# tho-kn/EgoTAP

Measured on AMD Instinct MI355X. Metric: stereo frames/sec (2D->3D lift, B=256, 256x256), higher is better.
Workload: dtype f32; 1 GPU; UnrealEgo 16-joint lifting head (heatmaps [B,90,64,64] -> joints [B,16,3]), forward only, fp32, batch 256 per GPU, inputs resident in HBM; batch_per_gpu=256, global_batch=256, heatmap=64, parallelism=dp1 (batch shards, no collective)

## Files before the change

### egotap_amd/csrc/egotap_abi.hip

```cpp
#include <stdarg.h>
#include <stdio.h>
#include <string.h>

#include <string>
#include <unordered_map>
#include <vector>

#include "attention_f32.h"
#include "common.h"
#include "conv_f32.h"
#include "conv_bf16.h"
#include "gemm_f32.h"
#include "gemm_bf16.h"
#include "gemm_bf16_dma.h"
#include "gemm_f32_dma.h"
#include "attention_bf16.h"
#include "layernorm.h"
#include "metrics.h"
#include "heatmap_synth.h"
#include "pu_chain.h"
#include "gemm_tn_bf16.h"
#include "train_ops.h"
#include "gemm_bf16s.h"
#include "gemm_bf16s64.h"
// ... 82 lines not shown
    const float *x2f0_w, *x2f0_b, *x2h0_w, *x2h0_b, *b2h0_w, *b2h0_b, *h2h0_w, *h2h0_b;
    const float *x2f1_w, *x2f1_b, *x2h1_w, *x2h1_b, *h2h1_w, *h2h1_b;
    const float *pose_w, *pose_b, *glob_w, *glob_b;
};

struct HmParams {
    struct Bn { const float *g, *b, *m, *v; long long* nbt; };
    const float* stem_w; Bn stem_bn;
    struct Block { const float *w1, *w2, *wd; Bn bn1, bn2, bnd; } blk[4][6];
    int nblk[4];
    struct Cv { const float *w, *b; } l1x1[4], up[3], head;
    int n_out;
};

struct egotap_handle_s {
    egotap_config cfg;
    int J, T, grid, ppd, side, seq, C, D, H, hid, out_joints;
    std::unordered_map<std::string, int64_t> expect[EGOTAP_NET_COUNT];
    std::unordered_map<std::string, Param> bound[EGOTAP_NET_COUNT];
    bool lift_resolved = false;
    LiftParams lp;
    std::unordered_map<std::string, Param> bound_grad;
    bool grad_resolved = false;
    LiftParams lg;
    bool hm_resolved[EGOTAP_NET_COUNT] = {false, false, false};
    HmParams hp[EGOTAP_NET_COUNT];
    int debug_stop = 0;
    int pu_resident[2] = {-1, -1};
    bool pu_chain = true;
    unsigned* pu_fault_host = nullptr;
    unsigned* pu_fault_dev = nullptr;
    int pu_faults = 0;
    int pu_debug_drop = 0;
    int precision = EGOTAP_PREC_F32;
    __bf16* wscratch = nullptr;
    size_t wscratch_bytes = 0;
    __bf16* ascratch = nullptr;
    size_t ascratch_bytes = 0;
    __bf16* conv_pack = nullptr;
    float* conv_part = nullptr;
    size_t conv_part_floats = 0;
    char* lift_arena = nullptr;
    char* hm_arena[EGOTAP_NET_COUNT] = {nullptr, nullptr, nullptr};
    short hm_arena_slab[EGOTAP_NET_COUNT][PackTable::MAXW] = {};
    int hm_arena_nw[EGOTAP_NET_COUNT] = {0, 0, 0};
    bool timing = false;
    std::vector<hipEvent_t> ev;
    struct Rec { const char* role; const char* kernel; double flops; };
    std::vector<Rec> rec;
    size_t ev_used = 0;
    std::string detail;
};
typedef egotap_handle_s Handle;

static int isqrt_floor(int v) {
    int r = 0;
    while ((r + 1) * (r + 1) <= v) ++r;
    return r;
}

static void lift_expect(Handle* h) {
    auto& e = h->expect[EGOTAP_NET_LIFT];
    const int64_t D = h->D, H = h->H, hid = h->hid, x = 2 * hid;
    const std::string v = "pos_heatmap_encoder.vit.";
    e[v + "embeddings.mask_token"] = D;
    e[v + "embeddings.position_embeddings"] = (int64_t)h->seq * D;
// ... 273 lines not shown
#endif
#if EGOTAP_IN(0)
extern "C" const char* egotap_timing_detail(egotap_handle h) { return h ? h->detail.c_str() : ""; }
#endif

struct GemmTimer {
    Handle* h;
    hipStream_t s;
    bool on;
    GemmTimer(Handle* h_, hipStream_t s_, const char* role, const char* kernel, double flops)
        : h(h_), s(s_), on(h_ && h_->timing) {
        if (!on) return;
        if (h->ev_used + 2 > h->ev.size()) {
            hipEvent_t a, b;
            if (hipEventCreate(&a) != hipSuccess || hipEventCreate(&b) != hipSuccess) { on = false; return; }
            h->ev.push_back(a);
            h->ev.push_back(b);
        }
        (void)hipEventRecord(h->ev[h->ev_used], s);
        h->rec.push_back({role, kernel, flops});
    }
    ~GemmTimer() {
        if (!on) return;
        (void)hipEventRecord(h->ev[h->ev_used + 1], s);
        h->ev_used += 2;
    }
};

template <class AL> struct AlName;
template <> struct AlName<ALoadPlain> { static constexpr const char* v = "ALoadPlain"; };
template <> struct AlName<ALoadPatch> { static constexpr const char* v = "ALoadPatch"; };
template <> struct AlName<ALoadTokens> { static constexpr const char* v = "ALoadTokens"; };
template <> struct AlName<ALoadLive> { static constexpr const char* v = "ALoadLive"; };
template <> struct AlName<ALoadRot> { static constexpr const char* v = "ALoadRot"; };
template <> struct AlName<ALoadStereo> { static constexpr const char* v = "ALoadStereo"; };
template <> struct AlName<ALoadStereoGated> { static constexpr const char* v = "ALoadStereoGated"; };
template <class E> struct EpiName;
template <> struct EpiName<EpiBias> { static constexpr const char* v = "EpiBias"; };
template <> struct EpiName<EpiBiasRes> { static constexpr const char* v = "EpiBiasRes"; };
template <> struct EpiName<EpiBiasResLive> { static constexpr const char* v = "EpiBiasResLive"; };
template <> struct EpiName<EpiBiasGelu> { static constexpr const char* v = "EpiBiasGelu"; };
template <> struct EpiName<EpiBnLrelu> { static constexpr const char* v = "EpiBnLrelu"; };
template <> struct EpiName<EpiPatch> { static constexpr const char* v = "EpiPatch"; };

template <class Cfg, class AL, class Epi>
static hipError_t gemm(Handle* h, const char* role, const AL& al, const SegMat& W, const Epi& epi, float* C, long ldc,
                       int M, int N, int K, hipStream_t s) {
    static const std::string kname = std::string("gemm_f32_kernel<") + std::to_string(Cfg::BM) + "x" +
                                     std::to_string(Cfg::BN) + "x" + std::to_string(Cfg::BK) + "," + AlName<AL>::v + "," +
                                     EpiName<Epi>::v + ">";
    GemmTimer t(h, s, role, kname.c_str(), 2.0 * M * N * K);
    return gemm_f32_launch<Cfg, AL, Epi>(al, W, epi, C, ldc, M, N, K, s);
}

static int device_cu_count() {
    static int n = 0;
    if (n == 0) {
        int dev = 0, v = 0;
        if (hipGetDevice(&dev) == hipSuccess && hipDeviceGetAttribute(&v, hipDeviceAttributeMultiprocessorCount, dev) == hipSuccess && v > 0) n = v;
        else n = 256;
    }
    return n;
}

static __global__ __launch_bounds__(256) void zero_fill_kernel(f32x4* __restrict__ p, long n16) {
    const long i = (long)blockIdx.x * blockDim.x + threadIdx.x;
    if (i < n16) p[i] = f32x4{0.f, 0.f, 0.f, 0.f};
}
static hipError_t zero_fill(void* p, size_t bytes, hipStream_t s) {
    if (bytes == 0) return hipSuccess;
    if ((((uintptr_t)p) | bytes) & 15) return hipErrorInvalidValue;
    const long n16 = (long)(bytes / 16);
    hipLaunchKernelGGL(zero_fill_kernel, dim3((unsigned)((n16 + 255) / 256)), dim3(256), 0, s, (f32x4*)p, n16);
    return hipGetLastError();
}

static __global__ __launch_bounds__(256) void concat3_kernel(const float* __restrict__ a, const float* __restrict__ b, const float* __restrict__ c,
                                                             float* __restrict__ out, int n) {
    const int i = blockIdx.x * blockDim.x + threadIdx.x;
    if (i < n) { out[i] = a[i]; out[n + i] = b[i]; out[2 * n + i] = c[i]; }
}

static __global__ __launch_bounds__(256) void f32_to_bf16_rows_kernel(const float* __restrict__ src, long lda, __bf16* __restrict__ dst, int k8, long n8) {
    const long i = (long)blockIdx.x * blockDim.x + threadIdx.x;
    if (i >= n8) return;
    const long row = i / k8;
    const float* p = src + row * lda + (i - row * k8) * 8;
    *(bf16x8*)(dst + i * 8) = bf16_round8(*(const f32x4*)p, *(const f32x4*)(p + 4));
}
template <class AL, class Epi>
static hipError_t gemm_bf16_plain(Handle* h, const AL& al, const SegMat& W, const Epi& epi, float* C, long ldc, int M, int N, int K, hipStream_t s) {
    const int nseg = N / W.seg;
    if (h && h->wscratch && (size_t)N * K * 2 <= h->wscratch_bytes && K % 8 == 0 && W.ld == K && nseg >= 1 && nseg <= 3 && nseg * W.seg == N) {
        SegMatB B;
        for (int i = 0; i < 3; ++i) B.p[i] = h->wscratch + (size_t)(i < nseg ? i : 0) * W.seg * K;
        B.seg = W.seg; B.ld = K;
        const long n8 = (long)W.seg * K / 8;
        for (int i = 0; i < nseg; ++i)
            hipLaunchKernelGGL(f32_to_bf16_kernel, dim3((unsigned)((n8 + 255) / 256)), dim3(256), 0, s, W.p[i], h->wscratch + (size_t)i * W.seg * K, n8);
        hipError_t e = hipGetLastError();
        if (e != hipSuccess) return e;
        if constexpr (std::is_same<AL, ALoadPlain>::value) {
            if (K % DmaCfg::BK == 0 && N % DmaCfg::BN == 0 && W.seg % DmaCfg::BN == 0 && al.lda % 4 == 0 && M >= 1024) {
                __bf16* a = (size_t)M * K * 2 <= h->ascratch_bytes ? h->ascratch : nullptr;
                if (a) {
                    const long a8 = (long)M * K / 8;
// ... 171 lines not shown
    EGO_CHECK(B >= 0, "negative batch");
    *bytes = lift_ws(h, B > 0 ? B : 1).total;
    return EGOTAP_OK;
}
#endif

#if EGOTAP_IN(0)
extern "C" int egotap_lift_intermediate(egotap_handle h, int B, const char* name, size_t* offset, int64_t* numel) {
    EGO_CHECK(h && name && offset && numel, "null argument");
    const LiftWs w = lift_ws(h, B > 0 ? B : 1);
    const int64_t M = (int64_t)B * h->seq;
    if (!strcmp(name, "tokens")) { *offset = w.Y; *numel = M * h->D; }
    else if (!strcmp(name, "x")) { *offset = w.X; *numel = M * h->D; }
    else if (!strcmp(name, "pos_embed")) { *offset = w.POSZ; *numel = (int64_t)B * h->T * h->hid; }
    else if (!strcmp(name, "rot_embed")) { *offset = w.ROTZ; *numel = (int64_t)B * h->T * h->hid; }
    else if (!strcmp(name, "skel_embed")) { *offset = w.HS1; *numel = (int64_t)h->J * B * h->H; }
    else { egotap_set_error("unknown intermediate '%s'", name); return EGOTAP_ERR_INVALID; }
    return EGOTAP_OK;
}
#endif

#if EGOTAP_IN(0)
extern "C" int egotap_set_pu_chain(egotap_handle h, int enable) {
    EGO_CHECK(h, "null handle");
    h->pu_chain = enable != 0;
    h->pu_resident[0] = h->pu_resident[1] = -1;
    return EGOTAP_OK;
}
extern "C" int egotap_debug_pu_drop_workgroups(egotap_handle h, int n) {
    EGO_CHECK(h && n >= 0 && n < 16, "egotap_debug_pu_drop_workgroups: n in [0, 16)");
    h->pu_debug_drop = n;
    return EGOTAP_OK;
}
extern "C" int egotap_pu_chain_status(egotap_handle h, int* enabled, int* faults) {
    EGO_CHECK(h, "null handle");
    if (h->pu_fault_host && __atomic_load_n(h->pu_fault_host, __ATOMIC_RELAXED) != 0u) {
        __atomic_store_n(h->pu_fault_host, 0u, __ATOMIC_RELAXED);
        h->pu_faults++;
        h->pu_chain = false;
        h->pu_resident[0] = h->pu_resident[1] = -1;
    }
    if (enabled) *enabled = h->pu_chain ? 1 : 0;
    if (faults) *faults = h->pu_faults;
    return EGOTAP_OK;
}
extern "C" int egotap_set_precision(egotap_handle h, int mode) {
    EGO_CHECK(h, "null handle");
    EGO_CHECK(mode == EGOTAP_PREC_F32 || mode == EGOTAP_PREC_BF16X3 || mode == EGOTAP_PREC_BF16, "egotap_set_precision: unknown mode %d", mode);
    h->precision = mode;
    h->lift_arena = nullptr;
    for (int n = 0; n < EGOTAP_NET_COUNT; ++n) h->hm_arena[n] = nullptr;
    return EGOTAP_OK;
}
#endif

#if EGOTAP_IN(0)
extern "C" int egotap_set_weight_scratch(egotap_handle h, void* buf, size_t bytes) {
    EGO_CHECK(h, "null handle");
    EGO_CHECK(((uintptr_t)buf & 15) == 0, "egotap_set_weight_scratch: 16-byte alignment");
    h->wscratch = (__bf16*)buf;
    h->wscratch_bytes = buf ? bytes : 0;
    return EGOTAP_OK;
}
#endif

#if EGOTAP_IN(0)
// ... 67 lines not shown
static EpiBiasResLive rebase(EpiBiasResLive e, int m0) { e.lr.m0 += m0; return e; }
template <class AL, class Epi>
static hipError_t gemm_rounds(Handle* h, const char* role, const AL& al, const SegMat& W, const Epi& epi, float* C, long ldc, int M, int N, int K,
                              hipStream_t s) {
    const int cus = device_cu_count(), tn = N / 256;
    const long tiles = (long)((M + 255) / 256) * tn;
    const int mh = (int)((tiles / cus) * cus / tn) * 256;
    if (N % 256 == 0 && K % 32 == 0 && mh > 0 && mh < M) {
        const double t_round = K * 0.2319 + 5.0;
        const double t_big = (double)((tiles + cus - 1) / cus) * t_round;
        const double t_split = (double)(((long)(mh / 256) * tn + cus - 1) / cus) * t_round + 4.0 + gemm_f32_direct_estimate_us<TileA>(M - mh, N, K, cus);
        if (t_split < t_big) {
            hipError_t e = gemm_big(h, role, al, W, epi, C, ldc, mh, N, K, s);
            if (e != hipSuccess) return e;
            return gemm<TileA>(h, role, rebase(al, mh), W, rebase(epi, mh), C + (long)mh * ldc, ldc, M - mh, N, K, s);
        }
    }
    return gemm_big(h, role, al, W, epi, C, ldc, M, N, K, s);
}

static bool lift_prune_last(Handle* h, int B) {
#ifdef EGOTAP_ATTN_F32_LIVE
    const int D = h->D, M = B * h->seq, Nq = h->T * h->ppd * h->ppd;
    if (h->precision != EGOTAP_PREC_F32 || h->debug_stop != 0 || h->cfg.vit_layers < 1 || Nq < 32 || Nq >= h->seq || D % 256 != 0) return false;
    const int cus = device_cu_count();
    if (gemm_small_route(h, true, M, 3 * D, D, D, cus, true).kind != GS_BIG || gemm_small_route(h, true, M, D, D, D, cus).kind != GS_BIG ||
        gemm_small_route(h, true, M, 4 * D, D, 4 * D, cus, true).kind != GS_BIG || gemm_small_route(h, true, M, D, 4 * D, D, cus).kind != GS_BIG)
        return false;
    return attention_f32_ksplit(B, h->seq, h->cfg.vit_heads, SPLITK_FLOATS, cus) == 1;
#else
    (void)h; (void)B;
    return false;
#endif
}

struct LiftFrozen {
    size_t patch, qkv[8], o[8], up[8], dn[8], bias3[8], fc1p, fc1r, total;
};
static bool lift_frozen_route(const Handle* h) { return h->precision == EGOTAP_PREC_BF16 && h->D == 1024 && h->seq % 32 == 0; }
static LiftFrozen lift_frozen_plan(const Handle* h, const LiftParams* p, PrepTable* T) {
    LiftFrozen f{};
    const size_t D = h->D, K1 = (size_t)h->ppd * h->ppd * D, K1r = 2 * (size_t)h->cfg.hm_size * h->cfg.hm_size;
    const int NL = h->cfg.vit_layers;
    size_t o = 0;
    int ns = 0;
    unsigned chunk = 0;
    auto seg = [&](const float* src, size_t elems, size_t elem_bytes, size_t at) {
        const size_t dst = at == (size_t)-1 ? o : at;
        if (at == (size_t)-1) o = al256(o + elems * elem_bytes);
        if (T && ns < PrepTable::MAXS) {
            T->s[ns] = PrepSeg{src, (unsigned long long)dst, (unsigned)(elems / 8), chunk};
            chunk += (unsigned)((elems / 8 + PrepTable::CHUNK8 - 1) / PrepTable::CHUNK8);
        }
        ++ns;
        return dst;
    };
    const size_t own = (size_t)-1;
    f.patch = seg(p ? p->patch_w : nullptr, D * 256, 2, own);
    for (int i = 0; i < NL; ++i) {
        const LiftParams::Layer* L = p ? &p->layer[i] : nullptr;
        f.qkv[i] = o;
        o = al256(o + 3 * D * D * 2);
        seg(L ? L->q_w : nullptr, D * D, 2, f.qkv[i]);
        seg(L ? L->k_w : nullptr, D * D, 2, f.qkv[i] + D * D * 2);
        seg(L ? L->v_w : nullptr, D * D, 2, f.qkv[i] + 2 * D * D * 2);
        f.o[i] = seg(L ? L->o_w : nullptr, D * D, 2, own);
// ... 101 lines not shown
            if (h->debug_stop == 2 + i) return EGOTAP_OK;
        }
        ln(p.lnf_g, p.lnf_b);
        auto bnf = [](const LiftParams::Fc& f, float* out) { return SEpiBnLreluF32{f.b, f.g, f.beta, f.mean, f.var, 1e-5f, 0.2f, out, 2048L}; };
        auto bn = [](const LiftParams::Fc& f) { return EpiBnLrelu{f.b, f.g, f.beta, f.mean, f.var, 1e-5f, 0.2f}; };
        {
            const int K1 = h->ppd * h->ppd * D;
            if (!frozen) prep(p.pos_fc[0].w, Wb, 2048, K1);
            const __bf16* W1 = frozen ? FW(fz.fc1p) : Wb;
            const XTokens xt{Yb, h->T, D, h->seq, h->side, h->ppd, h->grid};
            const int sp = gemm_bf16s_ksplit(BT, 2048, K1, cu, SPLITK_FLOATS);
            if (sp > 1) EGO_HIP(gemm_bf16s_splitk_launch(xt, W1, (long)K1, bnf(p.pos_fc[0], Z1), SPK, sp, BT, 2048, K1, cu, s));
            else EGO_HIP(fc1_nt(h, 0, Yb, W1, (long)K1, bnf(p.pos_fc[0], Z1), BT, cu, s));
            EGO_HIP((fc_gemm(h, "pos_fc2", ALoadPlain{Z1, 2048}, segmat1(p.pos_fc[1].w, 512, 2048), bn(p.pos_fc[1]), Z2, 512, BT, 512, 2048, SPK, s)));
            EGO_HIP((fc_gemm(h, "pos_fc3", ALoadPlain{Z2, 512}, segmat1(p.pos_fc[2].w, hid, 512), bn(p.pos_fc[2]), POSZ, hid, BT, hid, 512, SPK, s)));
        }
        {
            __bf16* hmb = HIDb;
            const long n8 = (long)B * h->C * HW / 8;
            hipLaunchKernelGGL(f32_to_bf16_kernel, dim3((unsigned)((n8 + 255) / 256)), dim3(256), 0, s, hm, hmb, n8);
            if (!frozen) prep(p.rot_fc[0].w, Wb, 2048, 2 * HW);
            const __bf16* W1 = frozen ? FW(fz.fc1r) : Wb;
            EGO_HIP(hipGetLastError());
            const XRot xr{hmb, h->C, J, HW};
            const int sp = gemm_bf16s_ksplit(BT, 2048, 2 * HW, cu, SPLITK_FLOATS);
            if (sp > 1) EGO_HIP(gemm_bf16s_splitk_launch(xr, W1, 2L * HW, bnf(p.rot_fc[0], Z1), SPK, sp, BT, 2048, 2 * HW, cu, s));
            else EGO_HIP(fc1_nt(h, 1, hmb, W1, 2L * HW, bnf(p.rot_fc[0], Z1), BT, cu, s));
            EGO_HIP((fc_gemm(h, "rot_fc2", ALoadPlain{Z1, 2048}, segmat1(p.rot_fc[1].w, 512, 2048), bn(p.rot_fc[1]), Z2, 512, BT, 512, 2048, SPK, s)));
            EGO_HIP((fc_gemm(h, "rot_fc3", ALoadPlain{Z2, 512}, segmat1(p.rot_fc[2].w, hid, 512), bn(p.rot_fc[2]), ROTZ, hid, BT, hid, 512, SPK, s)));
        }
    } else {
    const int NL = h->cfg.vit_layers;
    const bool prune = pose_only && lift_prune_last(h, B);
    EGO_HIP(launch_ln(X, Y, NL > 0 ? p.layer[0].ln1_g : p.lnf_g, NL > 0 ? p.layer[0].ln1_b : p.lnf_b, M, 1e-12f, s));
    for (int i = 0; i < NL; ++i) {
        const auto& L = p.layer[i];
#ifdef EGOTAP_ATTN_F32_LIVE
        if (prune && i + 1 == NL) {
            const LiveRows lr{h->seq, h->side, h->ppd, h->grid, h->T};
            const int Nq = h->T * h->ppd * h->ppd, Mc = B * Nq;
            float* Xc = QKV;
            SegMat Wkv; Wkv.p[0] = L.k_w; Wkv.p[1] = L.v_w; Wkv.p[2] = L.v_w; Wkv.seg = D; Wkv.ld = D;
            SegVec bkv; bkv.p[0] = L.k_b; bkv.p[1] = L.v_b; bkv.p[2] = L.v_b; bkv.seg = D;
            EGO_HIP((gemm_big(h, "kv", ALoadPlain{Y, D}, Wkv, EpiBias{bkv}, QKV + D, 3L * D, M, 2 * D, D, s)));
            EGO_HIP((gemm_rounds(h, "q_live", ALoadLive{Y, D, lr}, segmat1(L.q_w, D, D), EpiBias{segvec1(L.q_b, D)}, QKV, 3L * D, Mc, D, D, s)));
            EGO_HIP(attention_f32_live_launch(QKV, 3L * D, Nq, QKV, CTX, B, h->seq, h->cfg.vit_heads, s));
            EGO_HIP((gemm_rounds(h, "attn_out_live", ALoadPlain{CTX, D}, segmat1(L.o_w, D, D), EpiBiasResLive{segvec1(L.o_b, D), X, D, lr}, Xc, D, Mc, D, D, s)));
            EGO_HIP(launch_ln(Xc, Y, L.ln2_g, L.ln2_b, Mc, 1e-12f, s));
            EGO_HIP((gemm_rounds(h, "mlp_up_live", ALoadPlain{Y, D}, segmat1(L.up_w, 4 * D, D), EpiBiasGelu{segvec1(L.up_b, 4 * D)}, HID, 4L * D, Mc, 4 * D, D, s)));
            EGO_HIP((gemm_rounds(h, "mlp_down_live", ALoadPlain{HID, 4L * D}, segmat1(L.dn_w, D, 4 * D), EpiBiasRes{segvec1(L.dn_b, D), Xc, D}, Xc, D, Mc, D, 4 * D, s)));
            EGO_HIP(launch_ln(Xc, Y, p.lnf_g, p.lnf_b, Mc, 1e-12f, s));
            break;
        }
#endif
        {
            SegMat Wqkv; Wqkv.p[0] = L.q_w; Wqkv.p[1] = L.k_w; Wqkv.p[2] = L.v_w; Wqkv.seg = D; Wqkv.ld = D;
            SegVec bqkv; bqkv.p[0] = L.q_b; bqkv.p[1] = L.k_b; bqkv.p[2] = L.v_b; bqkv.seg = D;
            EGO_HIP((gemm_small(h, "qkv", ALoadPlain{Y, D}, Wqkv, EpiBias{bqkv}, QKV, 3L * D, M, 3 * D, D, SPK, s)));
        }
        if (h->precision == EGOTAP_PREC_BF16X3 && h->seq % 32 == 0) EGO_HIP(attention_bf16_launch<3>(QKV, CTX, B, h->seq, h->cfg.vit_heads, s));
        else if (h->precision == EGOTAP_PREC_BF16 && h->seq % 32 == 0) EGO_HIP(attention_bf16_launch<1>(QKV, CTX, B, h->seq, h->cfg.vit_heads, s));
        else EGO_HIP(attention_f32_launch(QKV, CTX, B, h->seq, h->cfg.vit_heads, s, nullptr, SPK, SPLITK_FLOATS, device_cu_count()));
        EGO_HIP(gemm_res_ln(h, "attn_out", CTX, D, L.o_w, L.o_b, X, M, D, D, L.ln2_g, L.ln2_b, Y, SPK, s));
        EGO_HIP((gemm_small(h, "mlp_up", ALoadPlain{Y, D}, segmat1(L.up_w, 4 * D, D), EpiBiasGelu{segvec1(L.up_b, 4 * D)}, HID, 4L * D, M, 4 * D, D, SPK, s)));
        const bool last = i + 1 == NL;
        EGO_HIP(gemm_res_ln(h, "mlp_down", HID, 4L * D, L.dn_w, L.dn_b, X, M, D, 4 * D, last ? p.lnf_g : p.layer[i + 1].ln1_g, last ? p.lnf_b : p.layer[i + 1].ln1_b, Y,
                            SPK, s));
        if (h->debug_stop == 2 + i) return EGOTAP_OK;
    }
    auto bn = [](const LiftParams::Fc& f) { return EpiBnLrelu{f.b, f.g, f.beta, f.mean, f.var, 1e-5f, 0.2f}; };
    const bool skinny_fc1 = BT < SKINNY_ROWS || (h->precision == EGOTAP_PREC_F32 && (long)((BT + 255) / 256) * (2048 / 256) < 100);
    {
        const int K1 = h->ppd * h->ppd * D;
        auto fc1 = [&](const auto& al) -> hipError_t {
            if (skinny_fc1 && BT <= 64)
                return gemm_f32_splitk_launch<TileS>(al, segmat1(p.pos_fc[0].w, 2048, K1), bn(p.pos_fc[0]), Z1, 2048, SPK, SPLITK_FLOATS, BT, 2048, K1, s, device_cu_count());
            if (skinny_fc1)
                return gemm_f32_splitk_launch<TileA>(al, segmat1(p.pos_fc[0].w, 2048, K1), bn(p.pos_fc[0]), Z1, 2048, SPK, SPLITK_FLOATS, BT, 2048, K1, s);
            return gemm_big(h, "pos_fc1", al, segmat1(p.pos_fc[0].w, 2048, K1), bn(p.pos_fc[0]), Z1, 2048, BT, 2048, K1, s);
        };
        if (prune) EGO_HIP(fc1(ALoadPlain{Y, (long)K1}));
        else EGO_HIP(fc1(ALoadTokens{Y, h->T, D, h->seq, h->side, h->ppd, h->grid}));
        EGO_HIP((fc_gemm(h, "pos_fc2", ALoadPlain{Z1, 2048}, segmat1(p.pos_fc[1].w, 512, 2048), bn(p.pos_fc[1]), Z2, 512, BT, 512, 2048, SPK, s)));
        EGO_HIP((fc_gemm(h, "pos_fc3", ALoadPlain{Z2, 512}, segmat1(p.pos_fc[2].w, hid, 512), bn(p.pos_fc[2]), POSZ, hid, BT, hid, 512, SPK, s)));
    }
    {
        ALoadRot al{hm, h->C, J, HW};
        if (skinny_fc1 && BT <= 64)
            EGO_HIP((gemm_f32_splitk_launch<TileS>(al, segmat1(p.rot_fc[0].w, 2048, 2L * HW), bn(p.rot_fc[0]), Z1, 2048, SPK, SPLITK_FLOATS, BT, 2048, 2 * HW, s, device_cu_count())));
        else if (skinny_fc1)
            EGO_HIP((gemm_f32_splitk_launch<TileA>(al, segmat1(p.rot_fc[0].w, 2048, 2L * HW), bn(p.rot_fc[0]), Z1, 2048, SPK, SPLITK_FLOATS, BT, 2048, 2 * HW, s)));
// ... 2636 lines not shown
```

### egotap_amd/csrc/gemm_f32.h

```cpp
#pragma once
#include "common.h"
#include <type_traits>

struct ALoadPlain {
    const float* A;
    long lda;
    struct Row { const float* p; };
    __device__ __forceinline__ Row row(int m) const { return Row{A + (long)m * lda}; }
    __device__ __forceinline__ f32x4 load(const Row& r, int k) const { return *(const f32x4*)(r.p + k); }
    static constexpr bool HAS_PTR = true;
    __device__ __forceinline__ const float* ptr(const Row& r, int k) const { return r.p + k; }
    __host__ bool dma_ok() const { return lda % 4 == 0 && lda < (1L << 21) && ((uintptr_t)A & 15) == 0; }
};

struct ALoadPatch {
    const float* hm;
    int C, S, seq, side, ppd, grid, T;
    const float* zeros = nullptr;
    struct Row { const float* p; };
    static constexpr bool HAS_PTR = true;
    __device__ __forceinline__ const float* ptr(const Row& r, int k) const { return r.p ? r.p + (k >> 4) * S + (k & 15) : zeros + k; }
    __host__ bool dma_ok() const { return zeros != nullptr && S % 4 == 0 && ((uintptr_t)hm & 15) == 0 && ((uintptr_t)zeros & 15) == 0; }
    __device__ __forceinline__ Row row(int m) const {
        const int b = m / seq, tok = m - b * seq;
// ... 23 lines not shown
    }
    static constexpr bool HAS_PTR = true;
    __device__ __forceinline__ const float* ptr(const Row& r, int k) const {
        const int s = k / D, c = k - s * D;
        const int prl = s / ppd, pcl = s - prl * ppd;
        return r.p + (long)(prl * side + pcl) * D + c;
    }
    __host__ bool dma_ok() const { return D % 4 == 0 && ((uintptr_t)Y & 15) == 0; }
};

struct LiveRows {
    int seq, side, ppd, grid, T;
    int m0 = 0;
    __host__ __device__ __forceinline__ long phys(int m) const {
        m += m0;
        const int pp = ppd * ppd, L = T * pp;
        const int b = m / L, r = m - b * L, i = r / pp, s = r - i * pp;
        const int pr = (i / grid) * ppd + s / ppd, pc = (i % grid) * ppd + s % ppd;
        return (long)b * seq + pr * side + pc;
    }
};
struct ALoadLive {
    const float* A;
    long lda;
    LiveRows lr;
    struct Row { const float* p; };
    __device__ __forceinline__ Row row(int m) const { return Row{A + lr.phys(m) * lda}; }
    __device__ __forceinline__ f32x4 load(const Row& r, int k) const { return *(const f32x4*)(r.p + k); }
    static constexpr bool HAS_PTR = true;
    __device__ __forceinline__ const float* ptr(const Row& r, int k) const { return r.p + k; }
    __host__ bool dma_ok() const { return lda % 4 == 0 && lda < (1L << 21) && ((uintptr_t)A & 15) == 0; }
};

struct ALoadRot {
    const float* hm;
    int C, J, HW;
    struct Row { const float* p; };
    __device__ __forceinline__ Row row(int m) const {
        const int T = 2 * J;
        const int b = m / T, t = m - b * T;
        const int eye = t / J, j = t - eye * J;
        return Row{hm + (long)(b * C + 2 * J + eye * 2 * J + j) * HW};
    }
    __device__ __forceinline__ f32x4 load(const Row& r, int k) const {
        const int cs = k / HW;
        return *(const f32x4*)(r.p + (long)cs * J * HW + (k - cs * HW));
    }
    static constexpr bool HAS_PTR = true;
    __device__ __forceinline__ const float* ptr(const Row& r, int k) const {
        const int cs = k / HW;
        return r.p + (long)cs * J * HW + (k - cs * HW);
    }
    __host__ bool dma_ok() const { return HW % 4 == 0 && ((uintptr_t)hm & 15) == 0; }
};

struct ALoadStereo {
    static constexpr bool HAS_PTR = false;
    const float* Z;
    int B, J, hid;
    struct Row { const float* p; };
    __device__ __forceinline__ Row row(int m) const {
        const int t = m / B, b = m - t * B;
        return Row{Z + ((long)b * 2 * J + t) * hid};
    }
    __device__ __forceinline__ f32x4 load(const Row& r, int k) const {
        const int eye = k / hid;
// ... 184 lines not shown
    struct Col4 {};
    __device__ __forceinline__ Col4 col4(int n0) const { return Col4{}; }
    static constexpr bool HAS_RES = true;
    __device__ __forceinline__ f32x4 res4(int m, int n0) const { return *(const f32x4*)(Z + (long)m * ldz + n0); }
    __device__ __forceinline__ f32x4 apply4(f32x4 acc, const Col4& c, f32x4 res, int m, int n0) const {
        f32x4 o;
#pragma unroll
        for (int i = 0; i < 4; ++i) o[i] = acc[i] * dgelu(res[i]);
        return o;
    }
};

struct EpiScatterPatch : EpiNone {
    float* hm;
    int C, S, seq, side, ppd, grid, T;
    __device__ __forceinline__ float* dst(int m, int n) const {
        const int b = m / seq, tok = m - b * seq;
        const int pr = tok / side, pc = tok - pr * side;
        const int cell = (pr / ppd) * grid + pc / ppd;
        if (cell >= T) return nullptr;
        return hm + ((long)(b * C + cell) * S + (pr % ppd) * 16 + (n >> 4)) * S + (pc % ppd) * 16 + (n & 15);
    }
};
struct EpiScatterRot : EpiNone {
    float* hm;
    int C, J, HW;
    __device__ __forceinline__ float* dst(int m, int n) const {
        const int T = 2 * J;
        const int b = m / T, t = m - b * T;
        const int eye = t / J, j = t - eye * J, cs = n / HW;
        return hm + (long)(b * C + 2 * J + eye * 2 * J + cs * J + j) * HW + (n - cs * HW);
    }
};
template <class E> struct epi_scatters : std::false_type {};
template <> struct epi_scatters<EpiScatterPatch> : std::true_type {};
template <> struct epi_scatters<EpiScatterRot> : std::true_type {};
template <class Epi>
__device__ __forceinline__ void epi_store(const Epi& epi, float* C, long ldc, int m, int n, float v) {
    if constexpr (epi_scatters<Epi>::value) {
        if (float* p = epi.dst(m, n)) *p = v;
    } else {
        C[(long)m * ldc + n] = v;
    }
}
template <class Epi>
__device__ __forceinline__ void epi_store4(const Epi& epi, float* C, long ldc, int m, int n0, const f32x4& v) {
    if constexpr (epi_scatters<Epi>::value) {
        if (float* p = epi.dst(m, n0)) *(f32x4*)p = v;
    } else {
        *(f32x4*)(C + (long)m * ldc + n0) = v;
    }
}

template <int BM_, int BN_, int BK_, int WM_, int WN_, int MINW_>
struct GemmCfg {
    static constexpr int BM = BM_, BN = BN_, BK = BK_, WM = WM_, WN = WN_, MINW = MINW_;
    static constexpr int THREADS = 64 * WM * WN;
    static constexpr int LDK = BK + 4;
    static constexpr int TM = BM / WM / 32, TN = BN / WN / 32;
    static constexpr int A_V4 = BM * BK / 4 / THREADS;
    static constexpr int B_V4 = BN * BK / 4 / THREADS;
    static constexpr int ROWS_PER_PASS = THREADS / (BK / 4);
    static constexpr int LDS_BYTES = 2 * (BM + BN) * LDK * 4;
    static_assert(BM % (32 * WM) == 0 && BN % (32 * WN) == 0, "wave tile must be a multiple of 32x32");
    static_assert(BK % 8 == 0, "BK multiple of 8");
    static_assert((BM * BK / 4) % THREADS == 0 && (BN * BK / 4) % THREADS == 0, "staging must divide evenly");
};

template <class Cfg, class ALoad, class Epi>
// ... 636 lines not shown
```

### egotap_amd/lib.py

```python
from __future__ import annotations

import ctypes as C
import os

from . import build as _build

ERR_NAMES = {1: "EGOTAP_ERR_INVALID", 2: "EGOTAP_ERR_HIP", 3: "EGOTAP_ERR_UNBOUND", 4: "EGOTAP_ERR_WORKSPACE"}
NET_LIFT, NET_HM_POS, NET_HM_ROT = 0, 1, 2
F32, I64 = 0, 1
PRECISIONS = {"f32": 0, "bf16x3": 1, "bf16": 2}


class EgotapConfig(C.Structure):
    _fields_ = [(n, C.c_int32) for n in (
        "struct_bytes", "n_joints_hm", "estimate_head", "hm_size", "hidden", "vit_dim", "vit_heads", "vit_layers",
        "patch", "pu_hidden")] + [("hm_blocks", C.c_int32 * 4)]


class EgotapError(RuntimeError):
    pass


_lib = None

_PROTOS = {
    "egotap_abi_version": (C.c_int, []),
    "egotap_last_error": (C.c_char_p, []),
    "egotap_create": (C.c_int, [C.POINTER(EgotapConfig), C.POINTER(C.c_void_p)]),
    "egotap_destroy": (None, [C.c_void_p]),
    "egotap_bind_param": (C.c_int, [C.c_void_p, C.c_int, C.c_char_p, C.c_void_p, C.c_int64, C.c_int]),
    "egotap_unbound_count": (C.c_int, [C.c_void_p, C.c_int, C.POINTER(C.c_int)]),
    "egotap_lift_workspace_bytes": (C.c_int, [C.c_void_p, C.c_int, C.POINTER(C.c_size_t)]),
    "egotap_lift_forward": (C.c_int, [C.c_void_p, C.c_void_p, C.c_int, C.c_void_p, C.c_void_p, C.c_size_t, C.c_void_p]),
    "egotap_lift_predict_pose": (C.c_int, [C.c_void_p, C.c_void_p, C.c_int, C.c_void_p, C.c_void_p, C.c_size_t, C.c_void_p]),
    "egotap_lift_intermediate": (C.c_int, [C.c_void_p, C.c_int, C.c_char_p, C.POINTER(C.c_size_t), C.POINTER(C.c_int64)]),
    "egotap_lift_debug_stop": (C.c_int, [C.c_void_p, C.c_int]),
    "egotap_set_precision": (C.c_int, [C.c_void_p, C.c_int]),
    "egotap_set_pu_chain": (C.c_int, [C.c_void_p, C.c_int]),
    "egotap_pu_chain_status": (C.c_int, [C.c_void_p, C.POINTER(C.c_int), C.POINTER(C.c_int)]),
    "egotap_debug_pu_drop_workgroups": (C.c_int, [C.c_void_p, C.c_int]),
    "egotap_debug_gemm_bk": (C.c_int, [C.c_int]),
    "egotap_debug_conv_addressing": (C.c_int, [C.c_int]),
    "egotap_set_weight_scratch": (C.c_int, [C.c_void_p, C.c_void_p, C.c_size_t]),
    "egotap_set_act_scratch": (C.c_int, [C.c_void_p, C.c_void_p, C.c_size_t]),
    "egotap_lift_frozen_bytes": (C.c_int, [C.c_void_p, C.POINTER(C.c_size_t)]),
    "egotap_lift_freeze": (C.c_int, [C.c_void_p, C.c_void_p, C.c_size_t, C.c_void_p]),
    "egotap_lift_unfreeze": (C.c_int, [C.c_void_p]),
    "egotap_hm_frozen_bytes": (C.c_int, [C.c_void_p, C.c_int, C.c_int, C.POINTER(C.c_size_t)]),
    "egotap_hm_freeze": (C.c_int, [C.c_void_p, C.c_int, C.c_int, C.c_void_p, C.c_size_t, C.c_void_p]),
    "egotap_hm_unfreeze": (C.c_int, [C.c_void_p, C.c_int]),
    "egotap_hm_workspace_bytes": (C.c_int, [C.c_void_p, C.c_int, C.POINTER(C.c_size_t)]),
    "egotap_hm_forward": (C.c_int, [C.c_void_p, C.c_int, C.c_void_p, C.c_void_p, C.c_int, C.c_void_p, C.c_int64, C.c_void_p,
                                    C.c_size_t, C.c_void_p]),
    "egotap_hm_intermediate": (C.c_int, [C.c_void_p, C.c_int, C.c_char_p, C.POINTER(C.c_size_t), C.POINTER(C.c_int64)]),
    "egotap_hm_forward_bnbatch_workspace_bytes": (C.c_int, [C.c_void_p, C.c_int, C.c_int, C.POINTER(C.c_size_t)]),
    "egotap_hm_forward_bnbatch_intermediate": (C.c_int, [C.c_void_p, C.c_int, C.c_int, C.c_char_p, C.POINTER(C.c_size_t), C.POINTER(C.c_int64)]),
    "egotap_hm_forward_bnbatch": (C.c_int, [C.c_void_p, C.c_int, C.c_void_p, C.c_void_p, C.c_int, C.c_void_p, C.c_int64, C.c_int, C.c_void_p,
                                            C.c_size_t, C.c_void_p]),
    "egotap_linear_f32": (C.c_int, [C.c_void_p] * 4 + [C.c_int] * 4 + [C.c_void_p] * 5 + [C.c_int, C.c_void_p]),
    "egotap_gemm_tile_name": (C.c_char_p, [C.c_int]),
    "egotap_linear_bf16_dma": (C.c_int, [C.c_void_p] * 4 + [C.c_int] * 3 + [C.c_void_p]),
    "egotap_layernorm_f32": (C.c_int, [C.c_void_p] * 4 + [C.c_int, C.c_int, C.c_float, C.c_void_p]),
    "egotap_attention_f32": (C.c_int, [C.c_void_p, C.c_void_p, C.c_int, C.c_int, C.c_int, C.c_void_p]),
    "egotap_pose_metrics": (C.c_int, [C.c_void_p, C.c_void_p, C.c_int, C.c_int, C.c_void_p, C.c_void_p, C.c_void_p, C.c_void_p]),
    "egotap_pose_metrics_batch_axes": (C.c_int, [C.c_void_p, C.c_void_p, C.c_int, C.c_int, C.c_void_p, C.c_void_p, C.c_void_p, C.c_void_p]),
    "egotap_attention": (C.c_int, [C.c_void_p, C.c_void_p, C.c_int, C.c_int, C.c_int, C.c_int, C.c_void_p]),
    "egotap_synth_heatmaps": (C.c_int, [C.c_void_p] * 4 + [C.c_int, C.c_int, C.c_int, C.c_void_p, C.c_void_p, C.c_void_p, C.c_void_p]),
    "egotap_timing_enable": (C.c_int, [C.c_void_p, C.c_int]),
    "egotap_timing_read": (C.c_int, [C.c_void_p, C.POINTER(C.c_int), C.POINTER(C.c_double), C.POINTER(C.c_double)]),
    "egotap_timing_detail": (C.c_char_p, [C.c_void_p]),
    "egotap_train_gemm_nt": (C.c_int, [C.c_void_p, C.c_int, C.c_void_p, C.c_int64, C.c_void_p, C.c_void_p, C.c_void_p, C.c_void_p,
                                       C.c_int, C.c_int, C.c_int, C.c_int, C.c_void_p, C.c_void_p, C.c_int, C.c_void_p]),
    "egotap_debug_wgrad_splits": (C.c_int, [C.c_int, C.c_int64, C.c_int64, C.c_size_t, C.c_int, C.c_int, C.c_double, C.c_double, C.POINTER(C.c_int)]),
# ... 213 lines not shown
```

### include/egotap_debug.h

```cpp
#ifndef EGOTAP_DEBUG_H
#define EGOTAP_DEBUG_H
#include "egotap.h"

#ifdef __cplusplus
extern "C" {
#endif

int egotap_debug_pu_drop_workgroups(egotap_handle h, int n);

int egotap_lift_debug_stop(egotap_handle h, int stage);

int egotap_debug_gemm_bk(int bk);

int egotap_debug_conv_addressing(int mode);

int egotap_debug_wgrad_splits(int tiles, int64_t slabs, int64_t n_floats, size_t slab_bytes, int num_cu, int lds_bytes, double slab_us, double fixed_us,
                              int* per);

int egotap_timing_enable(egotap_handle h, int enable);
int egotap_timing_read(egotap_handle h, int* launches, double* total_ms, double* total_flops);
const char* egotap_timing_detail(egotap_handle h);

#ifdef __cplusplus
}
#endif
#endif
```

Before: 2860 stereo frames/s.

## Compute layer-0 QKV for batch-invariant dummy token rows once and broadcast

In the first ViT layer of the lift head, tokens that do not depend on the input frame (dummy/padding patch rows past T) produce identical QKV across the batch. The layer-0 QKV GEMM now computes all live rows plus only one copy of the dummy rows, scattering results to their physical positions. A broadcast kernel then copies those rows to the other frames. This cuts the GEMM's M dimension, at the cost of an extra broadcast launch and scatter addressing in the load and epilogue.

```diff
diff --git a/egotap_amd/csrc/egotap_abi.hip b/egotap_amd/csrc/egotap_abi.hip
--- a/egotap_amd/csrc/egotap_abi.hip
+++ b/egotap_amd/csrc/egotap_abi.hip
@@ -138,6 +138,7 @@
     unsigned* pu_fault_dev = nullptr;
     int pu_faults = 0;
     int pu_debug_drop = 0;
+    bool shared_rows = true;
     int precision = EGOTAP_PREC_F32;
     __bf16* wscratch = nullptr;
     size_t wscratch_bytes = 0;
@@ -477,6 +478,7 @@
 template <> struct AlName<ALoadPatch> { static constexpr const char* v = "ALoadPatch"; };
 template <> struct AlName<ALoadTokens> { static constexpr const char* v = "ALoadTokens"; };
 template <> struct AlName<ALoadLive> { static constexpr const char* v = "ALoadLive"; };
+template <> struct AlName<ALoadShared> { static constexpr const char* v = "ALoadShared"; };
 template <> struct AlName<ALoadRot> { static constexpr const char* v = "ALoadRot"; };
 template <> struct AlName<ALoadStereo> { static constexpr const char* v = "ALoadStereo"; };
 template <> struct AlName<ALoadStereoGated> { static constexpr const char* v = "ALoadStereoGated"; };
@@ -484,6 +486,7 @@
 template <> struct EpiName<EpiBias> { static constexpr const char* v = "EpiBias"; };
 template <> struct EpiName<EpiBiasRes> { static constexpr const char* v = "EpiBiasRes"; };
 template <> struct EpiName<EpiBiasResLive> { static constexpr const char* v = "EpiBiasResLive"; };
+template <> struct EpiName<EpiBiasRows> { static constexpr const char* v = "EpiBiasRows"; };
 template <> struct EpiName<EpiBiasGelu> { static constexpr const char* v = "EpiBiasGelu"; };
 template <> struct EpiName<EpiBnLrelu> { static constexpr const char* v = "EpiBnLrelu"; };
 template <> struct EpiName<EpiPatch> { static constexpr const char* v = "EpiPatch"; };
@@ -517,6 +520,25 @@
     if ((((uintptr_t)p) | bytes) & 15) return hipErrorInvalidValue;
     const long n16 = (long)(bytes / 16);
     hipLaunchKernelGGL(zero_fill_kernel, dim3((unsigned)((n16 + 255) / 256)), dim3(256), 0, s, (f32x4*)p, n16);
+    return hipGetLastError();
+}
+
+static constexpr int BCAST_FRAMES = 8;
+static __global__ __launch_bounds__(256) void bcast_rows_kernel(float* C, long ld, SharedRows sr, int n_rows, int ld4, int seq, int B) {
+    const int i = blockIdx.x * 256 + threadIdx.x;
+    if (i >= n_rows * ld4) return;
+    const int d = i / ld4, c = i - d * ld4;
+    const long row = sr.phys(sr.n_live + d);
+    const f32x4 v = *(const f32x4*)(C + row * ld + c * 4);
+    const int b0 = 1 + blockIdx.y * BCAST_FRAMES, b1 = min(b0 + BCAST_FRAMES, B);
+    for (int b = b0; b < b1; ++b) *(f32x4*)(C + ((long)b * seq + row) * ld + c * 4) = v;
+}
+static hipError_t bcast_rows(float* C, long ld, const SharedRows& sr, int n_rows, int seq, int B, hipStream_t s) {
+    if (B < 2 || n_rows <= 0) return hipSuccess;
+    if (ld % 4 != 0 || ((uintptr_t)C & 15) != 0) return hipErrorInvalidValue;
+    const int ld4 = (int)(ld / 4);
+    hipLaunchKernelGGL(bcast_rows_kernel, dim3((unsigned)(((long)n_rows * ld4 + 255) / 256), (unsigned)((B - 1 + BCAST_FRAMES - 1) / BCAST_FRAMES)), dim3(256), 0, s,
+                       C, ld, sr, n_rows, ld4, seq, B);
     return hipGetLastError();
 }
 
@@ -754,6 +776,11 @@
     h->pu_debug_drop = n;
     return EGOTAP_OK;
 }
+extern "C" int egotap_debug_lift_shared_rows(egotap_handle h, int on) {
+    EGO_CHECK(h, "null handle");
+    h->shared_rows = on != 0;
+    return EGOTAP_OK;
+}
 extern "C" int egotap_pu_chain_status(egotap_handle h, int* enabled, int* faults) {
     EGO_CHECK(h, "null handle");
     if (h->pu_fault_host && __atomic_load_n(h->pu_fault_host, __ATOMIC_RELAXED) != 0u) {
@@ -887,6 +914,24 @@
     (void)h; (void)B;
     return false;
 #endif
+}
+
+static bool lift_shared_l0(Handle* h, int B) {
+    const int D = h->D, M = B * h->seq;
+    if (!h->shared_rows || h->precision != EGOTAP_PREC_F32 || h->cfg.vit_layers < 1 || h->T >= h->grid * h->grid || D % 256 != 0 || D >= (1 << 21) || B < 2)
+        return false;
+    return gemm_small_route(h, true, M, 3 * D, D, D, device_cu_count(), true).kind == GS_BIG;
+}
+static hipError_t qkv_shared_l0(Handle* h, const float* Y, const SegMat& W, const SegVec& bias, float* QKV, int B, hipStream_t s) {
+    const int D = h->D, Nq = h->T * h->ppd * h->ppd, n_dummy = h->seq - Nq, Ms = B * Nq + n_dummy;
+    const SharedRows sr{LiveRows{h->seq, h->side, h->ppd, h->grid, h->T}, B * Nq};
+    {
+        static const std::string kname = std::string("gemm_f32_dma_kernel<256x256x16,") + AlName<ALoadShared>::v + "," + EpiName<EpiBiasRows>::v + ">";
+        GemmTimer t(h, s, "qkv", kname.c_str(), 2.0 * Ms * 3 * D * D);
+        hipError_t e = gemm_f32_dma_launch(ALoadShared{Y, D, sr}, W, EpiBiasRows{{bias}, sr, QKV, 3L * D}, QKV, 3L * D, Ms, 3 * D, D, device_cu_count(), s);
+        if (e != hipSuccess) return e;
+    }
+    return bcast_rows(QKV, 3L * D, sr, n_dummy, h->seq, B, s);
 }
 
 struct LiftFrozen {
@@ -1054,6 +1099,7 @@
     } else {
     const int NL = h->cfg.vit_layers;
     const bool prune = pose_only && lift_prune_last(h, B);
+    const bool shared0 = lift_shared_l0(h, B);
     EGO_HIP(launch_ln(X, Y, NL > 0 ? p.layer[0].ln1_g : p.lnf_g, NL > 0 ? p.layer[0].ln1_b : p.lnf_b, M, 1e-12f, s));
     for (int i = 0; i < NL; ++i) {
         const auto& L = p.layer[i];
@@ -1078,7 +1124,8 @@
         {
             SegMat Wqkv; Wqkv.p[0] = L.q_w; Wqkv.p[1] = L.k_w; Wqkv.p[2] = L.v_w; Wqkv.seg = D; Wqkv.ld = D;
             SegVec bqkv; bqkv.p[0] = L.q_b; bqkv.p[1] = L.k_b; bqkv.p[2] = L.v_b; bqkv.seg = D;
-            EGO_HIP((gemm_small(h, "qkv", ALoadPlain{Y, D}, Wqkv, EpiBias{bqkv}, QKV, 3L * D, M, 3 * D, D, SPK, s)));
+            if (shared0 && i == 0) EGO_HIP(qkv_shared_l0(h, Y, Wqkv, bqkv, QKV, B, s));
+            else EGO_HIP((gemm_small(h, "qkv", ALoadPlain{Y, D}, Wqkv, EpiBias{bqkv}, QKV, 3L * D, M, 3 * D, D, SPK, s)));
         }
         if (h->precision == EGOTAP_PREC_BF16X3 && h->seq % 32 == 0) EGO_HIP(attention_bf16_launch<3>(QKV, CTX, B, h->seq, h->cfg.vit_heads, s));
         else if (h->precision == EGOTAP_PREC_BF16 && h->seq % 32 == 0) EGO_HIP(attention_bf16_launch<1>(QKV, CTX, B, h->seq, h->cfg.vit_heads, s));
diff --git a/egotap_amd/csrc/gemm_f32.h b/egotap_amd/csrc/gemm_f32.h
--- a/egotap_amd/csrc/gemm_f32.h
+++ b/egotap_amd/csrc/gemm_f32.h
@@ -79,6 +79,29 @@
     __host__ bool dma_ok() const { return lda % 4 == 0 && lda < (1L << 21) && ((uintptr_t)A & 15) == 0; }
 };
 
+struct SharedRows {
+    LiveRows lr;
+    int n_live;
+    __host__ __device__ __forceinline__ long phys(int m) const {
+        if (m < n_live) return lr.phys(m);
+        const int pp = lr.ppd * lr.ppd, d = m - n_live;
+        const int i = lr.T + d / pp, s = d - (d / pp) * pp;
+        const int pr = (i / lr.grid) * lr.ppd + s / lr.ppd, pc = (i % lr.grid) * lr.ppd + s % lr.ppd;
+        return (long)pr * lr.side + pc;
+    }
+};
+struct ALoadShared {
+    const float* A;
+    long lda;
+    SharedRows sr;
+    struct Row { const float* p; };
+    __device__ __forceinline__ Row row(int m) const { return Row{A + sr.phys(m) * lda}; }
+    __device__ __forceinline__ f32x4 load(const Row& r, int k) const { return *(const f32x4*)(r.p + k); }
+    static constexpr bool HAS_PTR = true;
+    __device__ __forceinline__ const float* ptr(const Row& r, int k) const { return r.p + k; }
+    __host__ bool dma_ok() const { return lda % 4 == 0 && lda < (1L << 21) && ((uintptr_t)A & 15) == 0; }
+};
+
 struct ALoadRot {
     const float* hm;
     int C, J, HW;
@@ -329,9 +352,16 @@
         return hm + (long)(b * C + 2 * J + eye * 2 * J + cs * J + j) * HW + (n - cs * HW);
     }
 };
+struct EpiBiasRows : EpiBias {
+    SharedRows sr;
+    float* C;
+    long ldc;
+    __device__ __forceinline__ float* dst(int m, int n) const { return C + sr.phys(m) * ldc + n; }
+};
 template <class E> struct epi_scatters : std::false_type {};
 template <> struct epi_scatters<EpiScatterPatch> : std::true_type {};
 template <> struct epi_scatters<EpiScatterRot> : std::true_type {};
+template <> struct epi_scatters<EpiBiasRows> : std::true_type {};
 template <class Epi>
 __device__ __forceinline__ void epi_store(const Epi& epi, float* C, long ldc, int m, int n, float v) {
     if constexpr (epi_scatters<Epi>::value) {
diff --git a/egotap_amd/lib.py b/egotap_amd/lib.py
--- a/egotap_amd/lib.py
+++ b/egotap_amd/lib.py
@@ -39,6 +39,7 @@
     "egotap_set_pu_chain": (C.c_int, [C.c_void_p, C.c_int]),
     "egotap_pu_chain_status": (C.c_int, [C.c_void_p, C.POINTER(C.c_int), C.POINTER(C.c_int)]),
     "egotap_debug_pu_drop_workgroups": (C.c_int, [C.c_void_p, C.c_int]),
+    "egotap_debug_lift_shared_rows": (C.c_int, [C.c_void_p, C.c_int]),
     "egotap_debug_gemm_bk": (C.c_int, [C.c_int]),
     "egotap_debug_conv_addressing": (C.c_int, [C.c_int]),
     "egotap_set_weight_scratch": (C.c_int, [C.c_void_p, C.c_void_p, C.c_size_t]),
diff --git a/include/egotap_debug.h b/include/egotap_debug.h
--- a/include/egotap_debug.h
+++ b/include/egotap_debug.h
@@ -9,6 +9,8 @@
 int egotap_debug_pu_drop_workgroups(egotap_handle h, int n);
 
 int egotap_lift_debug_stop(egotap_handle h, int stage);
+
+int egotap_debug_lift_shared_rows(egotap_handle h, int on);
 
 int egotap_debug_gemm_bk(int bk);
 
```

Result: no change. 2877 stereo frames/s (median of 6 runs) (+0.6%).
